# laomao0/BIN

Measured on NVIDIA H100. Metric: 720p frame-windows/sec, higher is better.
Workload: dtype f16

## Files before the change

### bin_b200/build.py

```python
from __future__ import annotations

import hashlib
import os
import subprocess
import sys
import tempfile

HERE = os.path.dirname(os.path.abspath(__file__))
CSRC = os.path.join(HERE, "csrc")
LIB = os.path.join(HERE, "libbin_b200.so")
SOURCES = ["conv_igemm.cu", "rdb_tail.cu", "aux_kernels.cu", "wgrad.cu", "metrics.cu", "png.cu", "api.cu"]
HEADERS = ["common.cuh", "wgmma.cuh", "xstack.cuh", "internal.h", os.path.join("..", "..", "include", "bin_b200.h")]
ARCH = ["-gencode", "arch=compute_90a,code=sm_90a"]
NVCC_FLAGS = [*ARCH, "-lineinfo", "-O3", "-std=c++17", "-Xcompiler", "-fPIC", "--expt-relaxed-constexpr", "-Xptxas", "-v"]


def _nvcc() -> str:
    for cand in (os.environ.get("NVCC"), "/usr/local/cuda/bin/nvcc", "nvcc"):
        if cand and (os.path.isabs(cand) and os.path.exists(cand) or not os.path.isabs(cand)):
            return cand
    raise RuntimeError("nvcc not found")


def _digest() -> str:
    h = hashlib.sha256()
    for f in SOURCES + HEADERS:
        with open(os.path.join(CSRC, f), "rb") as fh:
            h.update(fh.read())
    h.update(" ".join(NVCC_FLAGS).encode())
    return h.hexdigest()


def up_to_date(lib: str = LIB) -> bool:
    stamp = lib + ".sha256"
    return os.path.exists(lib) and os.path.exists(stamp) and open(stamp).read().strip() == _digest()


def build(force: bool = False, verbose: bool = False) -> str:
    stamp = LIB + ".sha256"
    dig = _digest()
    if not force and up_to_date():
        return LIB
    objs = []
    os.makedirs(os.path.join(HERE, "build"), exist_ok=True)
    procs = []
    for src in SOURCES:
        obj = os.path.join(HERE, "build", src.replace(".cu", ".o"))
        cmd = [_nvcc(), *NVCC_FLAGS, "-c", os.path.join(CSRC, src), "-o", obj]
        procs.append((src, subprocess.Popen(cmd, stdout=subprocess.PIPE, stderr=subprocess.STDOUT, text=True)))
        objs.append(obj)
    log = []
    for src, p in procs:
        out, _ = p.communicate()
        log.append(f"== {src}\n{out}")
        if p.returncode != 0:
            sys.stderr.write("\n".join(log))
            raise RuntimeError(f"nvcc failed on {src}")
    fd, tmp = tempfile.mkstemp(prefix=".libbin_b200.", suffix=".so", dir=HERE)
    os.close(fd)
    cmd = [_nvcc(), "-shared", "-o", tmp, *objs, *ARCH]
    r = subprocess.run(cmd, stdout=subprocess.PIPE, stderr=subprocess.STDOUT, text=True)
    log.append(r.stdout)
    if r.returncode != 0:
        os.unlink(tmp)
        sys.stderr.write("\n".join(log))
        raise RuntimeError("link failed")
    os.chmod(tmp, 0o755)
    os.replace(tmp, LIB)
    with open(os.path.join(HERE, "build", "nvcc.log"), "w") as fh:
        fh.write("\n".join(log))
    with open(stamp, "w") as fh:
        fh.write(dig)
    if verbose:
        print("\n".join(log))
    return LIB


if __name__ == "__main__":
    print(build(force="--force" in sys.argv, verbose=True))
```

### bin_b200/csrc/common.cuh

```cuda
#pragma once
#include <cuda.h>
#include <cuda_fp16.h>
#include <cuda_runtime.h>
#include <stdint.h>
#include <stdio.h>

#ifndef BIN_SPIN_LIMIT
#define BIN_SPIN_LIMIT (1u << 27)
#endif

namespace binb {

__device__ __forceinline__ uint32_t smem_u32(const void* p) {
  return static_cast<uint32_t>(__cvta_generic_to_shared(p));
}

__device__ __forceinline__ void mbar_init(uint64_t* bar, uint32_t count) {
  asm volatile("mbarrier.init.shared::cta.b64 [%0], %1;" ::"r"(smem_u32(bar)), "r"(count));
}
__device__ __forceinline__ void fence_barrier_init() {
  asm volatile("fence.mbarrier_init.release.cluster;" ::: "memory");
}
__device__ __forceinline__ void fence_proxy_async() {
  asm volatile("fence.proxy.async.shared::cta;" ::: "memory");
// ... 19 lines not shown
      : "memory");
  return ok != 0;
}
__device__ __forceinline__ void mbar_wait(uint64_t* bar, uint32_t parity) {
  uint32_t spins = 0;
  while (!mbar_try_wait(bar, parity)) {
    if (++spins > BIN_SPIN_LIMIT) {
__trap();
    }
  }
}

__device__ __forceinline__ void tma_prefetch_desc(const void* tmap) {
  asm volatile("prefetch.tensormap [%0];" ::"l"(tmap) : "memory");
}
__device__ __forceinline__ void tma_load_5d(void* smem_dst, const void* tmap, uint64_t* bar, int c0, int c1, int c2,
                                            int c3, int c4) {
  asm volatile(
      "cp.async.bulk.tensor.5d.shared::cluster.global.tile.mbarrier::complete_tx::bytes"
      " [%0], [%1, {%3, %4, %5, %6, %7}], [%2];" ::"r"(smem_u32(smem_dst)),
      "l"(tmap), "r"(smem_u32(bar)), "r"(c0), "r"(c1), "r"(c2), "r"(c3), "r"(c4)
      : "memory");
}
__device__ __forceinline__ void tma_load_4d(void* smem_dst, const void* tmap, uint64_t* bar, int c0, int c1, int c2,
                                            int c3) {
  asm volatile(
      "cp.async.bulk.tensor.4d.shared::cluster.global.tile.mbarrier::complete_tx::bytes"
      " [%0], [%1, {%3, %4, %5, %6}], [%2];" ::"r"(smem_u32(smem_dst)),
      "l"(tmap), "r"(smem_u32(bar)), "r"(c0), "r"(c1), "r"(c2), "r"(c3)
      : "memory");
}
__device__ __forceinline__ void bulk_load_1d(void* smem_dst, const void* gsrc, uint32_t bytes, uint64_t* bar) {
  asm volatile("cp.async.bulk.shared::cluster.global.mbarrier::complete_tx::bytes [%0], [%1], %2, [%3];" ::"r"(
                   smem_u32(smem_dst)),
               "l"(gsrc), "r"(bytes), "r"(smem_u32(bar))
               : "memory");
}

__device__ __forceinline__ uint64_t gmma_desc(uint32_t smem_addr, uint32_t lbo_bytes, uint32_t sbo_bytes) {
  return (uint64_t)((smem_addr >> 4) & 0x3FFFu) | ((uint64_t)((lbo_bytes >> 4) & 0x3FFFu) << 16) |
         ((uint64_t)((sbo_bytes >> 4) & 0x3FFFu) << 32);
}
__device__ __forceinline__ void wgmma_fence() { asm volatile("wgmma.fence.sync.aligned;" ::: "memory"); }
__device__ __forceinline__ void wgmma_commit() { asm volatile("wgmma.commit_group.sync.aligned;" ::: "memory"); }
template <int N>
__device__ __forceinline__ void wgmma_wait() { asm volatile("wgmma.wait_group.sync.aligned %0;" ::"n"(N) : "memory"); }
template <int K>
__device__ __forceinline__ void acc_fence(float (&d)[K]) {
#pragma unroll
  for (int i = 0; i < K; ++i) asm volatile("" : "+f"(d[i])::"memory");
}
__device__ __forceinline__ void wg_sync(int id) { asm volatile("bar.sync %0, 128;" ::"r"(id) : "memory"); }

}
```

### bin_b200/csrc/conv_igemm.cu

```cuda
#include <stdio.h>
#include <stdlib.h>

#include "common.cuh"
#include "internal.h"
#include "wgmma.cuh"
#include "xstack.cuh"

namespace binb {

template <int NT, int KS, bool SX>
struct ConvCfg {
  static constexpr int PAD = KS / 2;
  static constexpr int TW = kTWH - 2 * PAD;
  static constexpr bool ROWSPLIT = (KS == 5);
  static constexpr int ROWS = ROWSPLIT ? kTH : kTH + 2 * PAD;
  static constexpr int A_PLANE = ROWS * kTWH * 16;
  static constexpr int A_BYTES = kKPL * A_PLANE;
  static constexpr int NMMA = SX ? NT * KS : NT;
  static constexpr int TAPS_C = SX ? KS : KS * KS;
  static constexpr int TAPS_S = (SX || ROWSPLIT) ? KS : KS * KS;
  static constexpr int NSUB = ROWSPLIT ? KS : 1;
  static constexpr int W_TAP = kKPL * NMMA * 16;
  static constexpr int W_STAGE = TAPS_S * W_TAP;
  static constexpr int W_CHUNK = TAPS_C * W_TAP;
  static constexpr int XS_BYTES = SX ? kMT * 2 * 2 * kXsFloats<NT> * 4 : 0;
  static_assert(!(SX && ROWSPLIT), "SX is only used for 3x3");
  static_assert(NMMA % 16 == 0 && NMMA <= 256, "invalid wgmma N");
};

struct Ctrl {
  uint64_t full[kMaxStages];
  uint64_t empty[kMaxStages];
  uint64_t wfull[kMaxResidentChunks];
};
static_assert(sizeof(Ctrl) <= 1024, "ctrl block");

__device__ __forceinline__ uint32_t pack_h2(float a, float b) {
  __half2 h = __floats2half2_rn(a, b);
  return *reinterpret_cast<uint32_t*>(&h);
}
__device__ __forceinline__ float2 unpack_h2(uint32_t u) {
  __half2 h = *reinterpret_cast<__half2*>(&u);
  return __half22float2(h);
}

constexpr int kThreads = 384;

constexpr int kPsRowBytes = 4 * 16 + 16;
constexpr int kPsPartBytes = 4 * 8 * kPsRowBytes;
template <bool X3>
constexpr int kPsWarpBytes = (X3 ? 2 : 1) * kPsPartBytes;

__device__ __forceinline__ int x3_plane(int logical_plane) { return 2 * (logical_plane & ~3) + (logical_plane & 3); }
template <bool X3>
__device__ __forceinline__ void store_pair(__half* p, size_t lo_off, float a, float b) {
  if constexpr (X3) {
    const __half h0 = __float2half_rn(a), h1 = __float2half_rn(b);
    const __half2 hh = __halves2half2(h0, h1);
    *reinterpret_cast<__half2*>(p) = hh;
    *reinterpret_cast<__half2*>(p + lo_off) = __floats2half2_rn(a - __half2float(h0), b - __half2float(h1));
  } else {
    *reinterpret_cast<uint32_t*>(p) = pack_h2(a, b);
  }
}

template <int NT, int KS, int EPI, bool SX, bool X3>
__global__ void __launch_bounds__(kThreads, 1) conv_igemm_kernel(const __grid_constant__ ConvParams p) {
  using C = ConvCfg<NT, KS, SX>;
  static_assert(EPI != BIN_EPI_PIXSHUF || NT == 128, "the PixelShuffle staging buffer holds 4 output planes");
  constexpr int NA = C::NMMA / 2;
  auto tile_at = [&](int tq) { return p.reverse ? p.ntiles - 1 - tq : tq; };
  extern __shared__ __align__(1024) uint8_t smem[];
  Ctrl* ctrl = reinterpret_cast<Ctrl*>(smem);
  float* sbias = reinterpret_cast<float*>(smem + 1024);

  const int warp = __shfl_sync(0xffffffffu, threadIdx.x >> 5, 0);
  const int lane = threadIdx.x & 31;
  const uint32_t S = p.nstages;
  const int nchunks = p.nch0 + p.nch1;
  const int nunits = nchunks * C::NSUB;
  const int cps = p.cps;
  const int spt = (nunits + cps - 1) / cps;
  const int unit_bytes = C::A_BYTES + (p.resident ? 0 : C::W_STAGE);
  const int stage_bytes = cps * unit_bytes;
  uint8_t* res_w = smem + kCtrlBytes;
  uint8_t* stage0 = res_w + (p.resident ? nchunks * C::W_CHUNK : 0);

  if (threadIdx.x == 0) {
    tma_prefetch_desc(&p.tmap0);
    if (p.nch1 > 0) tma_prefetch_desc(&p.tmap1);
    for (int i = 0; i < kMaxStages; ++i) {
      mbar_init(&ctrl->full[i], 1);
      mbar_init(&ctrl->empty[i], 8);
    }
    for (int i = 0; i < kMaxResidentChunks; ++i) mbar_init(&ctrl->wfull[i], 1);
    fence_barrier_init();
  }
  const bool bias_in_smem = NT * p.nh <= 256;
  if (bias_in_smem)
    for (int i = threadIdx.x; i < NT * p.nh; i += blockDim.x) sbias[i] = p.bias[i];
  const float* bsrc = bias_in_smem ? sbias : p.bias;
  __syncthreads();

  if (warp == 0) {
    if (lane != 0) return;
    if (p.resident) {
      for (int c = 0; c < nchunks; ++c) {
        mbar_expect_tx(&ctrl->wfull[c], C::W_CHUNK);
        bulk_load_1d(res_w + c * C::W_CHUNK, reinterpret_cast<const uint8_t*>(p.w) + (size_t)c * C::W_CHUNK, C::W_CHUNK,
                     &ctrl->wfull[c]);
      }
    }
    uint32_t s = 0, ph = 0;
    for (int tq = blockIdx.x; tq < p.ntiles; tq += gridDim.x) {
      int t = tile_at(tq);
      const int nh = t % p.nh; t /= p.nh;
      const int txi = t % p.tiles_x; t /= p.tiles_x;
      const int tyi = t % p.tiles_y;
      const int b = p.b0 + t / p.tiles_y;
      const int x0 = txi * C::TW - C::PAD, y0 = p.y0 + tyi * kTH - C::PAD;
      int unit = 0;
      for (int j = 0; j < spt; ++j) {
        const int nu = (nunits - unit < cps) ? nunits - unit : cps;
        mbar_wait(&ctrl->empty[s], ph ^ 1);
        uint8_t* dst = stage0 + (size_t)s * stage_bytes;
        mbar_expect_tx(&ctrl->full[s], (uint32_t)(nu * unit_bytes));
        for (int u = 0; u < nu; ++u) {
          const int c = (unit + u) / C::NSUB, sub = (unit + u) % C::NSUB;
          const int lc = X3 ? c / 3 : c;
          const bool seg1 = lc >= p.nch0l;
          const void* tmap = seg1 ? (const void*)&p.tmap1 : (const void*)&p.tmap0;
          const int lplane = seg1 ? p.plane0_1 + (lc - p.nch0l) * kKPL : p.plane0_0 + lc * kKPL;
          const int plane = X3 ? 2 * lplane + ((c % 3) == 1 ? 4 : 0) : lplane;
          tma_load_4d(dst + (size_t)u * unit_bytes, tmap, &ctrl->full[s], x0 * 8, y0 + (C::ROWSPLIT ? sub : 0), plane, b);
          if (!p.resident) {
            const size_t woff = ((size_t)(nh * nchunks + c) * C::TAPS_C + (C::ROWSPLIT ? sub * KS : 0)) * C::W_TAP;
            bulk_load_1d(dst + (size_t)u * unit_bytes + C::A_BYTES, reinterpret_cast<const uint8_t*>(p.w) + woff,
                         C::W_STAGE, &ctrl->full[s]);
          }
        }
        unit += nu;
        if (++s == S) { s = 0; ph ^= 1; }
      }
    }
    return;
  }
  if (warp < 4) return;

  const int m = (warp - 4) >> 2;
  const int wq = warp & 3;
  const int k4 = lane & 3;
  float* xs = reinterpret_cast<float*>(stage0 + (size_t)S * stage_bytes) + (2 * m + (wq >> 1)) * 2 * kXsFloats<NT>;
  uint8_t* psbuf = stage0 + (size_t)S * stage_bytes + (warp - 4) * kPsWarpBytes<X3>;
  float acc[2][NA];
  constexpr float kAcc = X3 ? (1.f / 256.f) : 1.f;
  uint32_t s = 0, ph = 0;
  auto tile_coords = [&](int tq, int& nh, int& txi, int& tyi, int& b) {
    int t = tile_at(tq);
    nh = t % p.nh; t /= p.nh;
    txi = t % p.tiles_x; t /= p.tiles_x;
    tyi = t % p.tiles_y;
    b = p.b0 + t / p.tiles_y;
  };
  auto pixel = [&](int txi, int tyi, int mb, int h, int& y, int& x) {
    const int L = m * 128 + mb * 64 + wq * 16 + (lane >> 2) + 8 * h;
    const int ty = L >> 5, tx = L & 31;
    y = p.y0 + tyi * kTH + ty; x = txi * C::TW + tx;
    return (tx < C::TW) && (y < p.y0 + p.ny) && (x < p.W);
  };
  for (int tq = blockIdx.x; tq < p.ntiles; tq += gridDim.x) {
    constexpr int NFR = EPI == BIN_EPI_FINAL ? BIN_MAX_FRAMES : 1;
    float fpre[2][2][2][NFR];
    if constexpr (EPI == BIN_EPI_FINAL) {
      int nh, txi, tyi, b;
      tile_coords(tq, nh, txi, tyi, b);
      const int call = b / p.fr.Bc, bb = b % p.fr.Bc;
      const size_t hw = (size_t)p.H * p.W;
#pragma unroll
      for (int mb = 0; mb < 2; ++mb)
#pragma unroll
        for (int h = 0; h < 2; ++h) {
          int y, x;
          const bool valid = pixel(txi, tyi, mb, h, y, x);
#pragma unroll
          for (int e = 0; e < 2; ++e) {
            const int c = 2 * k4 + e;
            const size_t off = ((size_t)bb * 3 + c) * hw + (size_t)y * p.W + x;
#pragma unroll
            for (int fi = 0; fi < NFR; ++fi)
              fpre[mb][h][e][fi] = (valid && c < 3 && fi < p.fr.nframes) ? __ldg(p.fr.frame[call][fi] + off) : 0.f;
          }
        }
    }
    int unit = 0, prev = -1;
    for (int j = 0; j < spt; ++j) {
      const int nu = (nunits - unit < cps) ? nunits - unit : cps;
      mbar_wait(&ctrl->full[s], ph);
      if (p.resident && tq == (int)blockIdx.x) {
        for (int u = 0; u < nu; ++u)
          if ((unit + u) % C::NSUB == 0) mbar_wait(&ctrl->wfull[(unit + u) / C::NSUB], 0);
      }
      const uint32_t st_base = smem_u32(stage0 + (size_t)s * stage_bytes);
      wgmma_fence();
      for (int u = 0; u < nu; ++u) {
        const int c = (unit + u) / C::NSUB, sub = (unit + u) % C::NSUB;
        const uint32_t a_base = st_base + u * unit_bytes;
        const uint32_t w_base = p.resident ? smem_u32(res_w + c * C::W_CHUNK) + (C::ROWSPLIT ? sub * KS * C::W_TAP : 0)
                                           : a_base + C::A_BYTES;
        const uint32_t not_first = (unit + u) != 0 ? 1u : 0u;
#pragma unroll
        for (int tp = 0; tp < C::TAPS_S; ++tp) {
          const int ky = SX ? tp : (C::ROWSPLIT ? 0 : tp / KS);
          const int kx = SX ? 0 : (C::ROWSPLIT ? tp : tp % KS);
#pragma unroll
          for (int jj = 0; jj < kKC / 16; ++jj) {
            const uint64_t bd = gmma_desc(w_base + tp * C::W_TAP + jj * 2 * C::NMMA * 16, C::NMMA * 16, 128);
#pragma unroll
            for (int mb = 0; mb < 2; ++mb) {
              const uint32_t a_row = (uint32_t)(m * 128 + mb * 64 + ky * kTWH + kx);
              const uint64_t ad = gmma_desc(a_base + a_row * 16 + jj * 2 * C::A_PLANE, C::A_PLANE, 128);
              Wgmma<C::NMMA>::mma(acc[mb], ad, bd, (tp == 0 && jj == 0) ? not_first : 1u);
            }
          }
        }
      }
      wgmma_commit();
      wgmma_wait<1>();
      if (prev >= 0 && lane == 0) mbar_arrive(&ctrl->empty[prev]);
      prev = (int)s;
      unit += nu;
      if (++s == S) { s = 0; ph ^= 1; }
    }
    wgmma_wait<0>();
    acc_fence(acc[0]);
    acc_fence(acc[1]);
    if (lane == 0) mbar_arrive(&ctrl->empty[prev]);

    int nh, txi, tyi, b;
    tile_coords(tq, nh, txi, tyi, b);
#pragma unroll
    for (int mb = 0; mb < 2; ++mb) {
      if constexpr (SX) xstack_sum<NT>(acc[mb], xs + mb * kXsFloats<NT>, 3 + 2 * m + (wq >> 1));
#pragma unroll
      for (int h = 0; h < 2; ++h) {
        int y, x;
        const bool valid = pixel(txi, tyi, mb, h, y, x);
        auto val = [&](int i, int e) { return acc[mb][4 * i + 2 * h + e] * kAcc; };
        if constexpr (EPI == BIN_EPI_P8) {
          if (valid) {
            constexpr int NR = SX ? 1 : NT / 8;
            uint32_t rres[NR][X3 ? 2 : 1];
            if (!SX && p.res != nullptr) {
#pragma unroll
              for (int i = 0; i < NR; ++i) {
                const int rel = (nh * NT) / 8 + i;
                if (rel >= p.store_planes) continue;
                const int lp = p.res_plane0 + rel;
                const size_t off = ((((size_t)b * p.res_planes + (X3 ? x3_plane(lp) : lp)) * p.H + y) * p.W + x) * 8 + 2 * k4;
                rres[i][0] = *reinterpret_cast<const uint32_t*>(p.res + off);
                if constexpr (X3) rres[i][X3 ? 1 : 0] = *reinterpret_cast<const uint32_t*>(p.res + off + (size_t)4 * p.H * p.W * 8);
              }
            }
#pragma unroll
            for (int i = 0; i < NT / 8; ++i) {
              const int rel = (nh * NT) / 8 + i;
              if (rel >= p.store_planes) continue;
              const int n = nh * NT + 8 * i + 2 * k4;
              float f0 = val(i, 0) + bsrc[n], f1 = val(i, 1) + bsrc[n + 1];
              if (p.relu) { f0 = fmaxf(f0, 0.f); f1 = fmaxf(f1, 0.f); }
              if (!SX && p.res != nullptr) {
                const float2 g = unpack_h2(rres[SX ? 0 : i][0]);
                f0 += g.x; f1 += g.y;
                if constexpr (X3) {
                  const float2 g2 = unpack_h2(rres[SX ? 0 : i][X3 ? 1 : 0]);
                  f0 += g2.x; f1 += g2.y;
                }
              }
              const int op = p.out_plane0 + rel;
              const size_t off = ((((size_t)b * p.out_planes + (X3 ? x3_plane(op) : op)) * p.H + y) * p.W + x) * 8 + 2 * k4;
              store_pair<X3>(p.out + off, (size_t)4 * p.H * p.W * 8, f0, f1);
            }
          }
        } else if constexpr (EPI == BIN_EPI_PIXSHUF) {
          const int r = lane >> 2;
#pragma unroll
          for (int i = 0; i < NT / 8; ++i) {
#pragma unroll
            for (int e = 0; e < 2; ++e) {
              const int n = nh * NT + 8 * i + 2 * k4 + e;
              const float a = val(i, e) + sbias[n];
              const __half hi = __float2half_rn(a);
              __half* dst = reinterpret_cast<__half*>(psbuf + ((i >> 2) * 8 + r) * kPsRowBytes + (2 * (k4 & 1) + e) * 16) +
                            2 * (i & 3) + (k4 >> 1);
              dst[0] = hi;
              if constexpr (X3) dst[kPsPartBytes / 2] = __float2half_rn(a - __half2float(hi));
            }
          }
          __syncwarp();
          if (valid) {
            const int H2 = 2 * p.H, W2 = 2 * p.W;
            const int yy = 2 * y + (k4 >> 1), xx = 2 * x + (k4 & 1);
#pragma unroll
            for (int q = 0; q < NT / 32; ++q) {
              const int op = p.out_plane0 + nh * (NT / 32) + q;
              const size_t off = ((((size_t)b * p.out_planes + (X3 ? x3_plane(op) : op)) * H2 + yy) * W2 + xx) * 8;
#pragma unroll
              for (int part = 0; part < (X3 ? 2 : 1); ++part)
                *reinterpret_cast<uint4*>(p.out + off + (size_t)part * 4 * H2 * W2 * 8) =
                    *reinterpret_cast<const uint4*>(psbuf + part * kPsPartBytes + (q * 8 + r) * kPsRowBytes + k4 * 16);
            }
          }
          __syncwarp();
        } else {
          if (valid && k4 < 2) {
            const int call = b / p.fr.Bc, bb = b % p.fr.Bc;
            const size_t hw = (size_t)p.H * p.W;
#pragma unroll
            for (int e = 0; e < 2; ++e) {
              const int c = 2 * k4 + e;
              if (c >= 3) continue;
              const size_t off = ((size_t)bb * 3 + c) * hw + (size_t)y * p.W + x;
              float fm = fpre[mb][h][e][0];
#pragma unroll
              for (int fi = 1; fi < NFR; ++fi)
                if (fi < p.fr.nframes) fm += fpre[mb][h][e][fi];
              p.fr.out[call][off] = (val(0, e) + sbias[c]) + fm / (float)p.fr.nframes;
            }
          }
        }
      }
    }
  }
}

typedef CUresult (*EncodeTiledFn)(CUtensorMap*, CUtensorMapDataType, cuuint32_t, void*, const cuuint64_t*,
                                  const cuuint64_t*, const cuuint32_t*, const cuuint32_t*, CUtensorMapInterleave,
                                  CUtensorMapSwizzle, CUtensorMapL2promotion, CUtensorMapFloatOOBfill);

static EncodeTiledFn get_encode_fn() {
  static EncodeTiledFn fn = []() -> EncodeTiledFn {
    void* ptr = nullptr;
    cudaDriverEntryPointQueryResult q;
    if (cudaGetDriverEntryPoint("cuTensorMapEncodeTiled", &ptr, cudaEnableDefault, &q) != cudaSuccess ||
        q != cudaDriverEntryPointSuccess)
      return nullptr;
    return reinterpret_cast<EncodeTiledFn>(ptr);
  }();
  return fn;
}

int make_p8_tmap(CUtensorMap* m, const bin_act_t& t, int box_rows) {
  EncodeTiledFn fn = get_encode_fn();
  if (!fn) return fail(BIN_ERR_CUDA, "cuTensorMapEncodeTiled not available from the driver");
  if ((reinterpret_cast<uintptr_t>(t.ptr) & 15) != 0) return fail(BIN_ERR_ARG, "P8 tensor not 16-byte aligned");
  cuuint64_t dims[4] = {(cuuint64_t)t.W * 8, (cuuint64_t)t.H, (cuuint64_t)t.planes, (cuuint64_t)t.B};
  cuuint64_t strides[3] = {(cuuint64_t)t.W * 16, (cuuint64_t)t.H * t.W * 16, (cuuint64_t)t.planes * t.H * t.W * 16};
  cuuint32_t box[4] = {(cuuint32_t)kTWH * 8, (cuuint32_t)box_rows, (cuuint32_t)kKPL, 1};
  cuuint32_t estr[4] = {1, 1, 1, 1};
  CUresult r = fn(m, CU_TENSOR_MAP_DATA_TYPE_FLOAT16, 4, t.ptr, dims, strides, box, estr,
                  CU_TENSOR_MAP_INTERLEAVE_NONE, CU_TENSOR_MAP_SWIZZLE_NONE, CU_TENSOR_MAP_L2_PROMOTION_L2_256B,
                  CU_TENSOR_MAP_FLOAT_OOB_FILL_NONE);
  if (r != CUDA_SUCCESS) return fail(BIN_ERR_CUDA, "cuTensorMapEncodeTiled failed with code " + std::to_string((int)r));
  return BIN_OK;
}

int make_p8_tmap_box(CUtensorMap* m, const bin_act_t& t, int box_px, int box_rows, int box_planes) {
  EncodeTiledFn fn = get_encode_fn();
  if (!fn) return fail(BIN_ERR_CUDA, "cuTensorMapEncodeTiled not available from the driver");
  if ((reinterpret_cast<uintptr_t>(t.ptr) & 15) != 0) return fail(BIN_ERR_ARG, "P8 tensor not 16-byte aligned");
  if (box_px * 8 > 256 || box_rows > 256 || box_planes > 256) return fail(BIN_ERR_ARG, "TMA box dimension exceeds 256");
  cuuint64_t dims[4] = {(cuuint64_t)t.W * 8, (cuuint64_t)t.H, (cuuint64_t)t.planes, (cuuint64_t)t.B};
  cuuint64_t strides[3] = {(cuuint64_t)t.W * 16, (cuuint64_t)t.H * t.W * 16, (cuuint64_t)t.planes * t.H * t.W * 16};
  cuuint32_t box[4] = {(cuuint32_t)box_px * 8, (cuuint32_t)box_rows, (cuuint32_t)box_planes, 1};
  cuuint32_t estr[4] = {1, 1, 1, 1};
  CUresult r = fn(m, CU_TENSOR_MAP_DATA_TYPE_FLOAT16, 4, t.ptr, dims, strides, box, estr, CU_TENSOR_MAP_INTERLEAVE_NONE,
                  CU_TENSOR_MAP_SWIZZLE_NONE, CU_TENSOR_MAP_L2_PROMOTION_L2_256B, CU_TENSOR_MAP_FLOAT_OOB_FILL_NONE);
  if (r != CUDA_SUCCESS) return fail(BIN_ERR_CUDA, "cuTensorMapEncodeTiled failed with code " + std::to_string((int)r));
  return BIN_OK;
}

template <int NT, int KS, int EPI, bool SX, bool X3>
static int launch_inst(const bin_conv_args_t& a, cudaStream_t s, bool reverse) {
  using C = ConvCfg<NT, KS, SX>;
  ConvParams p;
// ... 78 lines not shown
  const int ny = a.y_count > 0 ? a.y_count : H - a.y_begin;
  if (a.b_begin < 0 || a.y_begin < 0 || a.b_count < 0 || a.y_count < 0 || nb < 1 || ny < 1 || a.b_begin + nb > B ||
      a.y_begin + ny > H)
    return fail(BIN_ERR_ARG, "conv: batch/row sub-range outside the tensor");
  if (a.epilogue != BIN_EPI_P8 && (a.relu || a.res.ptr))
    return fail(BIN_ERR_ARG, "conv: the pixel-shuffle and final epilogues take no ReLU and no residual");
  const bool sx = a.ksize == 3 && a.cout_pad == 32 && a.variant == BIN_CONV_DEFAULT;
  if (a.epilogue == BIN_EPI_P8) {
    const int nstore = a.store_planes > 0 ? a.store_planes : a.cout_pad / 8;
    if (a.out.H != H || a.out.W != W || a.out.B != B || nstore > a.cout_pad / 8 || plane_end(a.out_plane0, nstore) > a.out.planes)
      return fail(BIN_ERR_ARG, "conv: output tensor geometry mismatch");
    if (a.res.ptr && (a.res.H != H || a.res.W != W || a.res.B != B || plane_end(a.res_plane0, nstore) > a.res.planes))
      return fail(BIN_ERR_ARG, "conv: residual tensor geometry mismatch");
    if (sx && a.res.ptr) return fail(BIN_ERR_ARG, "conv: the x-stacked 3x3 / Cout 32 kernel takes no residual");
  } else if (a.epilogue == BIN_EPI_PIXSHUF) {
    if (a.out.H != 2 * H || a.out.W != 2 * W || a.out.B != B || plane_end(a.out_plane0, a.cout_pad / 32) > a.out.planes)
      return fail(BIN_ERR_ARG, "conv: pixel-shuffle output geometry mismatch");
    if (misaligned(a.out.ptr)) return fail(BIN_ERR_ARG, "conv: P8 tensor not 16-byte aligned");
  } else if (a.epilogue == BIN_EPI_FINAL) {
    if (a.fr.ncalls < 1 || a.fr.ncalls > BIN_MAX_CALLS || a.fr.nframes < 1 || a.fr.nframes > BIN_MAX_FRAMES ||
        a.fr.Bc < 1 || a.fr.ncalls * a.fr.Bc != B)
      return fail(BIN_ERR_ARG, "conv: frame table does not match the batch");
  }
  if (!a.in0.ptr || (has_in1 && !a.in1.ptr)) return fail(BIN_ERR_ARG, "conv: null input tensor");
  if (misaligned(a.in0.ptr) || (has_in1 && misaligned(a.in1.ptr))) return fail(BIN_ERR_ARG, "conv: P8 tensor not 16-byte aligned");
  if (!a.w_packed || !a.bias) return fail(BIN_ERR_ARG, "conv: null weights or bias");
  if (a.epilogue != BIN_EPI_FINAL && !a.out.ptr) return fail(BIN_ERR_ARG, "conv: null output tensor");
  if (a.epilogue == BIN_EPI_FINAL)
    for (int k = 0; k < a.fr.ncalls; ++k) {
      bool ok = a.fr.out[k] != nullptr;
      for (int fi = 0; fi < a.fr.nframes; ++fi) ok = ok && a.fr.frame[k][fi] != nullptr;
      if (!ok) return fail(BIN_ERR_ARG, "conv: null frame or output pointer in the frame table");
    }
  if (a.epilogue == BIN_EPI_P8) {
    if (sx) return launch_inst<32, 3, BIN_EPI_P8, true, X3>(a, s, reverse);
    if (a.ksize == 3 && a.cout_pad == 32 && a.variant == BIN_CONV_PLAIN && !X3) return launch_inst<32, 3, BIN_EPI_P8, false, false>(a, s, reverse);
    if (a.ksize == 3 && a.cout_pad % 96 == 0) return launch_inst<96, 3, BIN_EPI_P8, false, X3>(a, s, reverse);
    if (a.ksize == 5 && a.cout_pad == 96) return launch_inst<96, 5, BIN_EPI_P8, false, X3>(a, s, reverse);
    if (a.ksize == 1 && a.cout_pad % 96 == 0) return launch_inst<96, 1, BIN_EPI_P8, false, X3>(a, s, reverse);
  } else if (a.epilogue == BIN_EPI_PIXSHUF) {
    if (a.ksize == 3 && a.cout_pad == 256) return launch_inst<128, 3, BIN_EPI_PIXSHUF, false, X3>(a, s, reverse);
  } else if (a.epilogue == BIN_EPI_FINAL) {
    if (a.ksize == 3 && a.cout_pad == 16 && a.variant == BIN_CONV_DEFAULT) return launch_inst<16, 3, BIN_EPI_FINAL, true, X3>(a, s, reverse);
    if (a.ksize == 3 && a.cout_pad == 16 && a.variant == BIN_CONV_PLAIN && !X3) return launch_inst<16, 3, BIN_EPI_FINAL, false, false>(a, s, reverse);
  }
  return fail(BIN_ERR_UNSUPPORTED, "conv: no kernel instantiation for this conv (ksize/cout_pad/epilogue/precision)");
}

int launch_conv(const bin_conv_args_t& a, cudaStream_t s, bool reverse) {
  return a.x3 ? launch_conv_t<true>(a, s, reverse) : launch_conv_t<false>(a, s, reverse);
}

}
```

### bin_b200/csrc/rdb_tail.cu

```cuda
#include <stdio.h>
#include <stdlib.h>

#include "common.cuh"
#include "internal.h"
#include "wgmma.cuh"
#include "xstack.cuh"

namespace binb {

constexpr int kRtTH = 4;
constexpr int kRtRows = kRtTH + 2;
constexpr int kRtTW = kTWH - 2;
constexpr int kRtAPlane = kRtRows * kTWH * 16;
constexpr int kRtABytes = kKPL * kRtAPlane;
constexpr int kRtN = 96;
constexpr int kRtSlab = kKPL * kRtN * 16;
constexpr int kRtChunks = 6;
constexpr int kRtWChunk = 4 * kRtSlab;
constexpr int kRtWBytes = kRtChunks * kRtWChunk + kRtSlab;
constexpr int kRtHPlane = 128 * 16;
constexpr int kRtHBytes = kKPL * kRtHPlane;
constexpr int kRtXsBytes = 4 * kXsFloats<32> * 4;
constexpr int kRtCtrl = 1024;
constexpr int kRtStages = (kSmemMax - kRtCtrl - kRtWBytes - kRtHBytes - kRtXsBytes) / kRtABytes;
constexpr int kRtSmem = kRtCtrl + kRtWBytes + kRtHBytes + kRtStages * kRtABytes + kRtXsBytes;
static_assert(kRtStages >= 2 && kRtSmem <= kSmemMax, "rdb_tail shared memory");
static_assert((kRtCtrl + kRtWBytes + kRtHBytes) % 128 == 0 && kRtABytes % 128 == 0, "TMA destinations must be 128-byte aligned");

struct alignas(64) RdbTailParams {
  CUtensorMap tmap0, tmap1;
  int plane0_0, plane0_1;
  const uint8_t* w_conv;
  const uint8_t* w_lff;
  const float* b_conv;
  const float* b_lff;
  int H, W;
  int b0, y0, ny;
  int tiles_x, tiles_y, ntiles;
  __half* out; int out_planes, out_plane0;
  const __half* res; int res_planes, res_plane0;
  int reverse;
};

struct RtCtrl {
  uint64_t full[kRtStages], empty[kRtStages];
  uint64_t wfull[kRtChunks + 1];
};
static_assert(sizeof(RtCtrl) <= 512, "ctrl block");

__device__ __forceinline__ uint32_t pack_h2_rt(float a, float b) {
  __half2 h = __floats2half2_rn(a, b);
  return *reinterpret_cast<uint32_t*>(&h);
}
__device__ __forceinline__ float2 unpack_h2_rt(uint32_t u) {
  __half2 h = *reinterpret_cast<__half2*>(&u);
  return __half22float2(h);
}

__global__ void __launch_bounds__(384, 1) rdb_tail_kernel(const __grid_constant__ RdbTailParams p) {
  extern __shared__ __align__(1024) uint8_t smem[];
  RtCtrl* ctrl = reinterpret_cast<RtCtrl*>(smem);
  float* sb_conv = reinterpret_cast<float*>(smem + 512);
  float* sb_lff = sb_conv + 32;
  uint8_t* res_w = smem + kRtCtrl;
  uint8_t* htile = res_w + kRtWBytes;
  uint8_t* stage0 = htile + kRtHBytes;
  float* xs0 = reinterpret_cast<float*>(stage0 + kRtStages * kRtABytes);

  const int warp = __shfl_sync(0xffffffffu, threadIdx.x >> 5, 0);
  const int lane = threadIdx.x & 31;
  auto tile_of = [&](int tq, int& txi, int& tyi, int& b) {
    int t = p.reverse ? p.ntiles - 1 - tq : tq;
    txi = t % p.tiles_x; t /= p.tiles_x;
    tyi = t % p.tiles_y;
    b = p.b0 + t / p.tiles_y;
  };

  if (threadIdx.x == 0) {
    tma_prefetch_desc(&p.tmap0);
    tma_prefetch_desc(&p.tmap1);
    for (int i = 0; i < kRtStages; ++i) { mbar_init(&ctrl->full[i], 1); mbar_init(&ctrl->empty[i], 8); }
    for (int i = 0; i <= kRtChunks; ++i) mbar_init(&ctrl->wfull[i], 1);
    fence_barrier_init();
  }
  if (threadIdx.x < 32) sb_conv[threadIdx.x] = p.b_conv[threadIdx.x];
  else if (threadIdx.x < 128) sb_lff[threadIdx.x - 32] = p.b_lff[threadIdx.x - 32];
  __syncthreads();

  if (warp == 0) {
    if (lane != 0) return;
    for (int c = 0; c < kRtChunks; ++c) {
      mbar_expect_tx(&ctrl->wfull[c], kRtWChunk);
      bulk_load_1d(res_w + c * kRtWChunk, p.w_conv + (size_t)c * 3 * kRtSlab, 3 * kRtSlab, &ctrl->wfull[c]);
      bulk_load_1d(res_w + c * kRtWChunk + 3 * kRtSlab, p.w_lff + (size_t)c * kRtSlab, kRtSlab, &ctrl->wfull[c]);
    }
    mbar_expect_tx(&ctrl->wfull[kRtChunks], kRtSlab);
    bulk_load_1d(res_w + kRtChunks * kRtWChunk, p.w_lff + (size_t)kRtChunks * kRtSlab, kRtSlab, &ctrl->wfull[kRtChunks]);
    uint32_t s = 0, ph = 0;
    for (int tq = blockIdx.x; tq < p.ntiles; tq += gridDim.x) {
      int txi, tyi, b;
      tile_of(tq, txi, tyi, b);
      const int x0 = txi * kRtTW - 1, y0 = p.y0 + tyi * kRtTH - 1;
      for (int c = 0; c < kRtChunks; ++c) {
        mbar_wait(&ctrl->empty[s], ph ^ 1);
        mbar_expect_tx(&ctrl->full[s], kRtABytes);
        const bool seg1 = c >= 3;
        tma_load_4d(stage0 + (size_t)s * kRtABytes, seg1 ? (const void*)&p.tmap1 : (const void*)&p.tmap0, &ctrl->full[s],
                    x0 * 8, y0, seg1 ? p.plane0_1 + (c - 3) * kKPL : p.plane0_0 + c * kKPL, b);
        if (++s == kRtStages) { s = 0; ph ^= 1; }
      }
    }
    return;
  }
  if (warp < 4) return;

  const int m = (warp - 4) >> 2;
  const int wq = warp & 3;
  const int k4 = lane & 3;
  float* xs = xs0 + (2 * m + (wq >> 1)) * kXsFloats<32>;
  const int xs_bar = 3 + 2 * m + (wq >> 1);
  float acc_c[kRtN / 2], acc_l[kRtN / 2];
  uint32_t s = 0, ph = 0;
  for (int tq = blockIdx.x; tq < p.ntiles; tq += gridDim.x) {
    int prev = -1;
    for (int c = 0; c < kRtChunks; ++c) {
      mbar_wait(&ctrl->full[s], ph);
      if (tq == (int)blockIdx.x) mbar_wait(&ctrl->wfull[c], 0);
      const uint32_t a_base = smem_u32(stage0 + (size_t)s * kRtABytes) + m * 64 * 16;
      const uint32_t b_base = smem_u32(res_w + c * kRtWChunk);
      const uint32_t first = c == 0 ? 0u : 1u;
      wgmma_fence();
#pragma unroll
      for (int ky = 0; ky < 3; ++ky) {
#pragma unroll
        for (int jj = 0; jj < kKC / 16; ++jj)
          Wgmma<kRtN>::mma(acc_c, gmma_desc(a_base + ky * kTWH * 16 + jj * 2 * kRtAPlane, kRtAPlane, 128),
                           gmma_desc(b_base + ky * kRtSlab + jj * 2 * kRtN * 16, kRtN * 16, 128),
                           (jj == 0 && ky == 0) ? first : 1u);
      }
#pragma unroll
      for (int jj = 0; jj < kKC / 16; ++jj)
        Wgmma<kRtN>::mma(acc_l, gmma_desc(a_base + (kTWH + 1) * 16 + jj * 2 * kRtAPlane, kRtAPlane, 128),
                         gmma_desc(b_base + 3 * kRtSlab + jj * 2 * kRtN * 16, kRtN * 16, 128), jj == 0 ? first : 1u);
      wgmma_commit();
      wgmma_wait<1>();
      if (prev >= 0 && lane == 0) mbar_arrive(&ctrl->empty[prev]);
      prev = (int)s;
      if (++s == kRtStages) { s = 0; ph ^= 1; }
    }
    wgmma_wait<0>();
    acc_fence(acc_c);
    acc_fence(acc_l);
    if (lane == 0) mbar_arrive(&ctrl->empty[prev]);

    int txi, tyi, b;
    tile_of(tq, txi, tyi, b);
    bool valid[2];
    int y[2], x[2];
    uint32_t res[2][kRtN / 8];
#pragma unroll
    for (int h = 0; h < 2; ++h) {
      const int L = m * 64 + wq * 16 + (lane >> 2) + 8 * h;
      y[h] = p.y0 + tyi * kRtTH + (L >> 5);
      x[h] = txi * kRtTW + (L & 31);
      valid[h] = (L & 31) < kRtTW && y[h] < p.y0 + p.ny && x[h] < p.W;
#pragma unroll
      for (int i = 0; i < kRtN / 8; ++i) {
        const size_t roff = ((((size_t)b * p.res_planes + p.res_plane0 + i) * p.H + y[h]) * p.W + x[h]) * 8 + 2 * k4;
        res[h][i] = valid[h] ? *reinterpret_cast<const uint32_t*>(p.res + roff) : 0u;
      }
    }

    xstack_sum<32>(acc_c, xs, xs_bar);
#pragma unroll
    for (int h = 0; h < 2; ++h) {
      const int r = wq * 16 + (lane >> 2) + 8 * h;
      uint8_t* hrow = htile + (m * 64 + r) * 16 + 4 * k4;
#pragma unroll
      for (int i = 0; i < 4; ++i) {
        float f[2];
#pragma unroll
        for (int e = 0; e < 2; ++e) f[e] = fmaxf(acc_c[4 * i + 2 * h + e] + sb_conv[8 * i + 2 * k4 + e], 0.f);
        *reinterpret_cast<uint32_t*>(hrow + i * kRtHPlane) = pack_h2_rt(f[0], f[1]);
      }
    }
    fence_proxy_async();
    wg_sync(1 + m);

    if (tq == (int)blockIdx.x) mbar_wait(&ctrl->wfull[kRtChunks], 0);
    wgmma_fence();
    {
      const uint32_t h_base = smem_u32(htile) + m * 64 * 16;
      const uint32_t b_base = smem_u32(res_w + kRtChunks * kRtWChunk);
#pragma unroll
      for (int jj = 0; jj < kKC / 16; ++jj)
        Wgmma<kRtN>::mma(acc_l, gmma_desc(h_base + jj * 2 * kRtHPlane, kRtHPlane, 128),
                         gmma_desc(b_base + jj * 2 * kRtN * 16, kRtN * 16, 128), 1u);
    }
    wgmma_commit();
    wgmma_wait<0>();
    acc_fence(acc_l);

#pragma unroll
    for (int h = 0; h < 2; ++h) {
      if (valid[h]) {
#pragma unroll
        for (int i = 0; i < kRtN / 8; ++i) {
          const int n = 8 * i + 2 * k4;
          const float2 g = unpack_h2_rt(res[h][i]);
          const size_t off = ((((size_t)b * p.out_planes + p.out_plane0 + i) * p.H + y[h]) * p.W + x[h]) * 8 + 2 * k4;
          *reinterpret_cast<uint32_t*>(p.out + off) =
              pack_h2_rt((acc_l[4 * i + 2 * h] + sb_lff[n]) + g.x, (acc_l[4 * i + 2 * h + 1] + sb_lff[n + 1]) + g.y);
        }
      }
    }
    wg_sync(1 + m);
  }
}

int make_p8_tmap(CUtensorMap* m, const bin_act_t& t, int box_rows);

int launch_rdb_tail(const bin_act_t& x, int x_plane0, const bin_act_t& g, int g_plane0, const void* w_conv,
                    const float* b_conv, const void* w_lff, const float* b_lff, const bin_act_t& out, int out_plane0,
                    int b_begin, int b_count, int y_begin, int y_count, cudaStream_t s, bool reverse) {
  const int H = x.H, W = x.W, B = x.B;
  if (g.H != H || g.W != W || g.B != B || out.H != H || out.W != W || out.B != B)
    return fail(BIN_ERR_ARG, "rdb_tail: tensor geometry mismatch");
  if (x_plane0 < 0 || g_plane0 < 0 || out_plane0 < 0 || x_plane0 + 12 > x.planes || g_plane0 + 12 > g.planes ||
      out_plane0 + 12 > out.planes)
    return fail(BIN_ERR_ARG, "rdb_tail: plane range exceeds tensor");
  RdbTailParams p;
  memset(&p, 0, sizeof(p));
  p.plane0_0 = x_plane0; p.plane0_1 = g_plane0;
  p.w_conv = reinterpret_cast<const uint8_t*>(w_conv); p.w_lff = reinterpret_cast<const uint8_t*>(w_lff);
  p.b_conv = b_conv; p.b_lff = b_lff;
  p.H = H; p.W = W;
  p.b0 = b_begin; p.y0 = y_begin;
  const int nb = b_count > 0 ? b_count : B - b_begin;
  p.ny = y_count > 0 ? y_count : H - y_begin;
  if (p.b0 < 0 || p.y0 < 0 || nb < 1 || p.ny < 1 || p.b0 + nb > B || p.y0 + p.ny > H)
    return fail(BIN_ERR_ARG, "rdb_tail: batch/row sub-range outside the tensor");
  if (!x.ptr || !g.ptr || !out.ptr || !w_conv || !b_conv || !w_lff || !b_lff) return fail(BIN_ERR_ARG, "rdb_tail_fwd: null argument");
  p.tiles_x = (W + kRtTW - 1) / kRtTW;
  p.tiles_y = (p.ny + kRtTH - 1) / kRtTH;
  p.ntiles = nb * p.tiles_x * p.tiles_y;
  p.out = reinterpret_cast<__half*>(out.ptr); p.out_planes = out.planes; p.out_plane0 = out_plane0;
  p.res = reinterpret_cast<const __half*>(x.ptr); p.res_planes = x.planes; p.res_plane0 = x_plane0;
  p.reverse = reverse ? 1 : 0;
  BIN_TRY(make_p8_tmap(&p.tmap0, x, kRtRows));
  BIN_TRY(make_p8_tmap(&p.tmap1, g, kRtRows));
  static std::atomic<unsigned long long> opted{0};
  BIN_TRY(ensure_dynamic_smem(rdb_tail_kernel, kRtSmem, opted));
  const int sms = num_sms();
  const int grid = p.ntiles < sms ? p.ntiles : sms;
  rdb_tail_kernel<<<grid, 384, kRtSmem, s>>>(p);
  BIN_CUDA_OK(cudaGetLastError());
  return BIN_OK;
}

}
```

Before: 15.51.

## Overlap next-tile conv head with RDB tail epilogue and read residual from smem

In the RDB tail kernel, the first two conv chunks of the next tile are issued before waiting on the LFF GEMM, so tensor-core work overlaps the epilogue stores. The residual is read from the staged TMA input tile in shared memory instead of a separate global load. Both kernels also hand registers from producer to consumer warpgroups with setmaxnreg. Optional clock64 phase instrumentation is added behind a compile flag, along with a build helper for instrumented libraries. This adds ring-slot ordering constraints and raises register pressure in the consumers.

New measurement: 16.70, median of 6. 1.08x the previous value.

```diff
diff --git a/bin_b200/build.py b/bin_b200/build.py
--- a/bin_b200/build.py
+++ b/bin_b200/build.py
@@ -36,17 +36,13 @@
     return os.path.exists(lib) and os.path.exists(stamp) and open(stamp).read().strip() == _digest()
 
 
-def build(force: bool = False, verbose: bool = False) -> str:
-    stamp = LIB + ".sha256"
-    dig = _digest()
-    if not force and up_to_date():
-        return LIB
+def _compile_link(lib: str, obj_dir: str, extra_flags: list) -> str:
     objs = []
-    os.makedirs(os.path.join(HERE, "build"), exist_ok=True)
+    os.makedirs(obj_dir, exist_ok=True)
     procs = []
     for src in SOURCES:
-        obj = os.path.join(HERE, "build", src.replace(".cu", ".o"))
-        cmd = [_nvcc(), *NVCC_FLAGS, "-c", os.path.join(CSRC, src), "-o", obj]
+        obj = os.path.join(obj_dir, src.replace(".cu", ".o"))
+        cmd = [_nvcc(), *NVCC_FLAGS, *extra_flags, "-c", os.path.join(CSRC, src), "-o", obj]
         procs.append((src, subprocess.Popen(cmd, stdout=subprocess.PIPE, stderr=subprocess.STDOUT, text=True)))
         objs.append(obj)
     log = []
@@ -56,7 +52,7 @@
         if p.returncode != 0:
             sys.stderr.write("\n".join(log))
             raise RuntimeError(f"nvcc failed on {src}")
-    fd, tmp = tempfile.mkstemp(prefix=".libbin_b200.", suffix=".so", dir=HERE)
+    fd, tmp = tempfile.mkstemp(prefix=".libbin_b200.", suffix=".so", dir=os.path.dirname(lib))
     os.close(fd)
     cmd = [_nvcc(), "-shared", "-o", tmp, *objs, *ARCH]
     r = subprocess.run(cmd, stdout=subprocess.PIPE, stderr=subprocess.STDOUT, text=True)
@@ -66,14 +62,29 @@
         sys.stderr.write("\n".join(log))
         raise RuntimeError("link failed")
     os.chmod(tmp, 0o755)
-    os.replace(tmp, LIB)
+    os.replace(tmp, lib)
+    return "\n".join(log)
+
+
+def build(force: bool = False, verbose: bool = False) -> str:
+    stamp = LIB + ".sha256"
+    dig = _digest()
+    if not force and up_to_date():
+        return LIB
+    log = _compile_link(LIB, os.path.join(HERE, "build"), [])
     with open(os.path.join(HERE, "build", "nvcc.log"), "w") as fh:
-        fh.write("\n".join(log))
+        fh.write(log)
     with open(stamp, "w") as fh:
         fh.write(dig)
     if verbose:
-        print("\n".join(log))
+        print(log)
     return LIB
+
+
+def build_instrumented(out_dir: str, defines: list) -> str:
+    lib = os.path.join(out_dir, "libbin_b200_" + "_".join(d.lower() for d in defines) + ".so")
+    _compile_link(lib, os.path.join(out_dir, "obj"), [f"-D{d}" for d in defines])
+    return lib
 
 
 if __name__ == "__main__":
diff --git a/bin_b200/csrc/common.cuh b/bin_b200/csrc/common.cuh
--- a/bin_b200/csrc/common.cuh
+++ b/bin_b200/csrc/common.cuh
@@ -95,4 +95,22 @@
 }
 __device__ __forceinline__ void wg_sync(int id) { asm volatile("bar.sync %0, 128;" ::"r"(id) : "memory"); }
 
+constexpr int kProducerRegs = 40;
+constexpr int kConsumerRegs = 232;
+template <int R>
+__device__ __forceinline__ void setmaxnreg_dec() { asm volatile("setmaxnreg.dec.sync.aligned.u32 %0;" ::"n"(R)); }
+template <int R>
+__device__ __forceinline__ void setmaxnreg_inc() { asm volatile("setmaxnreg.inc.sync.aligned.u32 %0;" ::"n"(R)); }
+
+#ifdef BIN_RDB_PHASES
+#define BIN_PH(...) __VA_ARGS__
+struct PhaseBuf {
+  unsigned long long* rec;
+  int max_tiles;
+};
+enum { PH_START, PH_LAST_FULL, PH_MMA_DONE, PH_EPI_DONE, PH_STARVED_MAIN, PH_STARVED_EPI, kPhTile = 8 };
+#else
+#define BIN_PH(...)
+#endif
+
 }
diff --git a/bin_b200/csrc/conv_igemm.cu b/bin_b200/csrc/conv_igemm.cu
--- a/bin_b200/csrc/conv_igemm.cu
+++ b/bin_b200/csrc/conv_igemm.cu
@@ -44,6 +44,10 @@
   return __half22float2(h);
 }
 
+#ifdef BIN_RDB_PHASES
+static __device__ PhaseBuf g_ph_conv;
+#endif
+
 constexpr int kThreads = 384;
 
 constexpr int kPsRowBytes = 4 * 16 + 16;
@@ -68,6 +72,7 @@
 __global__ void __launch_bounds__(kThreads, 1) conv_igemm_kernel(const __grid_constant__ ConvParams p) {
   using C = ConvCfg<NT, KS, SX>;
   static_assert(EPI != BIN_EPI_PIXSHUF || NT == 128, "the PixelShuffle staging buffer holds 4 output planes");
+  constexpr bool kRdb = SX && EPI == BIN_EPI_P8;
   constexpr int NA = C::NMMA / 2;
   auto tile_at = [&](int tq) { return p.reverse ? p.ntiles - 1 - tq : tq; };
   extern __shared__ __align__(1024) uint8_t smem[];
@@ -102,8 +107,10 @@
   const float* bsrc = bias_in_smem ? sbias : p.bias;
   __syncthreads();
 
-  if (warp == 0) {
-    if (lane != 0) return;
+  if (warp < 4) {
+    if constexpr (kRdb) setmaxnreg_dec<kProducerRegs>();
+    if (warp != 0 || lane != 0) return;
+    BIN_PH(unsigned long long blocked = 0, ntq = 0;)
     if (p.resident) {
       for (int c = 0; c < nchunks; ++c) {
         mbar_expect_tx(&ctrl->wfull[c], C::W_CHUNK);
@@ -122,7 +129,9 @@
       int unit = 0;
       for (int j = 0; j < spt; ++j) {
         const int nu = (nunits - unit < cps) ? nunits - unit : cps;
+        BIN_PH(const unsigned long long w0 = clock64();)
         mbar_wait(&ctrl->empty[s], ph ^ 1);
+        BIN_PH(blocked += clock64() - w0;)
         uint8_t* dst = stage0 + (size_t)s * stage_bytes;
         mbar_expect_tx(&ctrl->full[s], (uint32_t)(nu * unit_bytes));
         for (int u = 0; u < nu; ++u) {
@@ -142,10 +151,15 @@
         unit += nu;
         if (++s == S) { s = 0; ph ^= 1; }
       }
-    }
+      BIN_PH(++ntq;)
+    }
+    BIN_PH(if (kRdb && g_ph_conv.rec) {
+      g_ph_conv.rec[2 * (size_t)g_ph_conv.max_tiles * kPhTile + 2 * blockIdx.x] = blocked;
+      g_ph_conv.rec[2 * (size_t)g_ph_conv.max_tiles * kPhTile + 2 * blockIdx.x + 1] = ntq;
+    })
     return;
   }
-  if (warp < 4) return;
+  if constexpr (kRdb) setmaxnreg_inc<kConsumerRegs>();
 
   const int m = (warp - 4) >> 2;
   const int wq = warp & 3;
@@ -168,7 +182,10 @@
     y = p.y0 + tyi * kTH + ty; x = txi * C::TW + tx;
     return (tx < C::TW) && (y < p.y0 + p.ny) && (x < p.W);
   };
+  BIN_PH(const bool rec = kRdb && wq == 0 && lane == 0 && g_ph_conv.rec != nullptr;
+         unsigned long long starved = 0, starved_main = 0, t_start = 0, t_last_full = 0, t_mma = 0;)
   for (int tq = blockIdx.x; tq < p.ntiles; tq += gridDim.x) {
+    BIN_PH(t_start = clock64();)
     constexpr int NFR = EPI == BIN_EPI_FINAL ? BIN_MAX_FRAMES : 1;
     float fpre[2][2][2][NFR];
     if constexpr (EPI == BIN_EPI_FINAL) {
@@ -195,11 +212,13 @@
     int unit = 0, prev = -1;
     for (int j = 0; j < spt; ++j) {
       const int nu = (nunits - unit < cps) ? nunits - unit : cps;
+      BIN_PH(const unsigned long long w0 = clock64();)
       mbar_wait(&ctrl->full[s], ph);
       if (p.resident && tq == (int)blockIdx.x) {
         for (int u = 0; u < nu; ++u)
           if ((unit + u) % C::NSUB == 0) mbar_wait(&ctrl->wfull[(unit + u) / C::NSUB], 0);
       }
+      BIN_PH(starved += clock64() - w0;)
       const uint32_t st_base = smem_u32(stage0 + (size_t)s * stage_bytes);
       wgmma_fence();
       for (int u = 0; u < nu; ++u) {
@@ -231,10 +250,12 @@
       unit += nu;
       if (++s == S) { s = 0; ph ^= 1; }
     }
+    BIN_PH(t_last_full = clock64();)
     wgmma_wait<0>();
     acc_fence(acc[0]);
     acc_fence(acc[1]);
     if (lane == 0) mbar_arrive(&ctrl->empty[prev]);
+    BIN_PH(t_mma = clock64(); starved_main = starved; starved = 0;)
 
     int nh, txi, tyi, b;
     tile_coords(tq, nh, txi, tyi, b);
@@ -330,6 +351,11 @@
         }
       }
     }
+    BIN_PH(if (rec && tq < g_ph_conv.max_tiles) {
+      unsigned long long* r = g_ph_conv.rec + (2 * (size_t)tq + m) * kPhTile;
+      r[PH_START] = t_start; r[PH_LAST_FULL] = t_last_full; r[PH_MMA_DONE] = t_mma; r[PH_EPI_DONE] = clock64();
+      r[PH_STARVED_MAIN] = starved_main; r[PH_STARVED_EPI] = starved;
+    } starved = 0;)
   }
 }
 
@@ -514,3 +540,10 @@
 }
 
 }
+
+#ifdef BIN_RDB_PHASES
+extern "C" int bin_rdb_phases_arm_conv(void* rec, int max_tiles) {
+  const binb::PhaseBuf b{reinterpret_cast<unsigned long long*>(rec), max_tiles};
+  return cudaMemcpyToSymbol(binb::g_ph_conv, &b, sizeof(b)) == cudaSuccess ? BIN_OK : BIN_ERR_CUDA;
+}
+#endif
diff --git a/bin_b200/csrc/rdb_tail.cu b/bin_b200/csrc/rdb_tail.cu
--- a/bin_b200/csrc/rdb_tail.cu
+++ b/bin_b200/csrc/rdb_tail.cu
@@ -16,6 +16,7 @@
 constexpr int kRtN = 96;
 constexpr int kRtSlab = kKPL * kRtN * 16;
 constexpr int kRtChunks = 6;
+constexpr int kRtXChunks = 3;
 constexpr int kRtWChunk = 4 * kRtSlab;
 constexpr int kRtWBytes = kRtChunks * kRtWChunk + kRtSlab;
 constexpr int kRtHPlane = 128 * 16;
@@ -25,6 +26,9 @@
 constexpr int kRtStages = (kSmemMax - kRtCtrl - kRtWBytes - kRtHBytes - kRtXsBytes) / kRtABytes;
 constexpr int kRtSmem = kRtCtrl + kRtWBytes + kRtHBytes + kRtStages * kRtABytes + kRtXsBytes;
 static_assert(kRtStages >= 2 && kRtSmem <= kSmemMax, "rdb_tail shared memory");
+constexpr int kRtHead = 2;
+static_assert(kRtHead >= 1 && kRtHead < kRtChunks && kRtHead <= kRtStages,
+              "the head's ring slots must be released by the main loop of the tile before");
 static_assert((kRtCtrl + kRtWBytes + kRtHBytes) % 128 == 0 && kRtABytes % 128 == 0, "TMA destinations must be 128-byte aligned");
 
 struct alignas(64) RdbTailParams {
@@ -38,7 +42,6 @@
   int b0, y0, ny;
   int tiles_x, tiles_y, ntiles;
   __half* out; int out_planes, out_plane0;
-  const __half* res; int res_planes, res_plane0;
   int reverse;
 };
 
@@ -56,6 +59,10 @@
   __half2 h = *reinterpret_cast<__half2*>(&u);
   return __half22float2(h);
 }
+
+#ifdef BIN_RDB_PHASES
+static __device__ PhaseBuf g_ph_tail;
+#endif
 
 __global__ void __launch_bounds__(384, 1) rdb_tail_kernel(const __grid_constant__ RdbTailParams p) {
   extern __shared__ __align__(1024) uint8_t smem[];
@@ -87,8 +94,10 @@
   else if (threadIdx.x < 128) sb_lff[threadIdx.x - 32] = p.b_lff[threadIdx.x - 32];
   __syncthreads();
 
-  if (warp == 0) {
-    if (lane != 0) return;
+  if (warp < 4) {
+    setmaxnreg_dec<kProducerRegs>();
+    if (warp != 0 || lane != 0) return;
+    BIN_PH(unsigned long long blocked = 0, ntq = 0;)
     for (int c = 0; c < kRtChunks; ++c) {
       mbar_expect_tx(&ctrl->wfull[c], kRtWChunk);
       bulk_load_1d(res_w + c * kRtWChunk, p.w_conv + (size_t)c * 3 * kRtSlab, 3 * kRtSlab, &ctrl->wfull[c]);
@@ -102,17 +111,24 @@
       tile_of(tq, txi, tyi, b);
       const int x0 = txi * kRtTW - 1, y0 = p.y0 + tyi * kRtTH - 1;
       for (int c = 0; c < kRtChunks; ++c) {
+        BIN_PH(const unsigned long long w0 = clock64();)
         mbar_wait(&ctrl->empty[s], ph ^ 1);
+        BIN_PH(blocked += clock64() - w0;)
         mbar_expect_tx(&ctrl->full[s], kRtABytes);
-        const bool seg1 = c >= 3;
+        const bool seg1 = c >= kRtXChunks;
         tma_load_4d(stage0 + (size_t)s * kRtABytes, seg1 ? (const void*)&p.tmap1 : (const void*)&p.tmap0, &ctrl->full[s],
-                    x0 * 8, y0, seg1 ? p.plane0_1 + (c - 3) * kKPL : p.plane0_0 + c * kKPL, b);
+                    x0 * 8, y0, seg1 ? p.plane0_1 + (c - kRtXChunks) * kKPL : p.plane0_0 + c * kKPL, b);
         if (++s == kRtStages) { s = 0; ph ^= 1; }
       }
-    }
+      BIN_PH(++ntq;)
+    }
+    BIN_PH(if (g_ph_tail.rec) {
+      g_ph_tail.rec[2 * (size_t)g_ph_tail.max_tiles * kPhTile + 2 * blockIdx.x] = blocked;
+      g_ph_tail.rec[2 * (size_t)g_ph_tail.max_tiles * kPhTile + 2 * blockIdx.x + 1] = ntq;
+    })
     return;
   }
-  if (warp < 4) return;
+  setmaxnreg_inc<kConsumerRegs>();
 
   const int m = (warp - 4) >> 2;
   const int wq = warp & 3;
@@ -121,54 +137,90 @@
   const int xs_bar = 3 + 2 * m + (wq >> 1);
   float acc_c[kRtN / 2], acc_l[kRtN / 2];
   uint32_t s = 0, ph = 0;
+  BIN_PH(const bool rec = wq == 0 && lane == 0 && g_ph_tail.rec != nullptr;
+         unsigned long long starved = 0, starved_main = 0, t_start = 0, t_last_full = 0, t_mma = 0;)
+  auto a_base_of = [&](uint32_t slot) { return smem_u32(stage0 + (size_t)slot * kRtABytes) + m * 64 * 16; };
+  auto conv_mma = [&](uint32_t a_base, int c) {
+    const uint32_t b_base = smem_u32(res_w + c * kRtWChunk);
+#pragma unroll
+    for (int ky = 0; ky < 3; ++ky)
+#pragma unroll
+      for (int jj = 0; jj < kKC / 16; ++jj)
+        Wgmma<kRtN>::mma(acc_c, gmma_desc(a_base + ky * kTWH * 16 + jj * 2 * kRtAPlane, kRtAPlane, 128),
+                         gmma_desc(b_base + ky * kRtSlab + jj * 2 * kRtN * 16, kRtN * 16, 128),
+                         (jj == 0 && ky == 0 && c == 0) ? 0u : 1u);
+  };
+  auto issue_head = [&](bool exists, bool first_tile) {
+    uint32_t hs = s, hph = ph;
+#pragma unroll
+    for (int c = 0; c < kRtHead; ++c) {
+      if (exists) {
+        BIN_PH(const unsigned long long w0 = clock64();)
+        mbar_wait(&ctrl->full[hs], hph);
+        if (first_tile) mbar_wait(&ctrl->wfull[c], 0);
+        BIN_PH(starved += clock64() - w0;)
+      }
+      wgmma_fence();
+      conv_mma(a_base_of(hs), c);
+      if (++hs == kRtStages) { hs = 0; hph ^= 1; }
+    }
+    wgmma_commit();
+  };
+
+  issue_head(true, true);
   for (int tq = blockIdx.x; tq < p.ntiles; tq += gridDim.x) {
+    const bool first_tile = tq == (int)blockIdx.x;
+    BIN_PH(t_start = clock64();)
+    uint32_t res[2][kRtN / 8];
     int prev = -1;
+#pragma unroll
     for (int c = 0; c < kRtChunks; ++c) {
-      mbar_wait(&ctrl->full[s], ph);
-      if (tq == (int)blockIdx.x) mbar_wait(&ctrl->wfull[c], 0);
-      const uint32_t a_base = smem_u32(stage0 + (size_t)s * kRtABytes) + m * 64 * 16;
+      if (c >= kRtHead) {
+        BIN_PH(const unsigned long long w0 = clock64();)
+        mbar_wait(&ctrl->full[s], ph);
+        if (first_tile) mbar_wait(&ctrl->wfull[c], 0);
+        BIN_PH(starved += clock64() - w0;)
+      }
+      const uint32_t a_base = a_base_of(s);
+      wgmma_fence();
+      if (c >= kRtHead) conv_mma(a_base, c);
       const uint32_t b_base = smem_u32(res_w + c * kRtWChunk);
-      const uint32_t first = c == 0 ? 0u : 1u;
-      wgmma_fence();
-#pragma unroll
-      for (int ky = 0; ky < 3; ++ky) {
-#pragma unroll
-        for (int jj = 0; jj < kKC / 16; ++jj)
-          Wgmma<kRtN>::mma(acc_c, gmma_desc(a_base + ky * kTWH * 16 + jj * 2 * kRtAPlane, kRtAPlane, 128),
-                           gmma_desc(b_base + ky * kRtSlab + jj * 2 * kRtN * 16, kRtN * 16, 128),
-                           (jj == 0 && ky == 0) ? first : 1u);
-      }
 #pragma unroll
       for (int jj = 0; jj < kKC / 16; ++jj)
         Wgmma<kRtN>::mma(acc_l, gmma_desc(a_base + (kTWH + 1) * 16 + jj * 2 * kRtAPlane, kRtAPlane, 128),
-                         gmma_desc(b_base + 3 * kRtSlab + jj * 2 * kRtN * 16, kRtN * 16, 128), jj == 0 ? first : 1u);
+                         gmma_desc(b_base + 3 * kRtSlab + jj * 2 * kRtN * 16, kRtN * 16, 128), (jj == 0 && c == 0) ? 0u : 1u);
       wgmma_commit();
+      if (c < kRtXChunks) {
+#pragma unroll
+        for (int h = 0; h < 2; ++h)
+#pragma unroll
+          for (int j = 0; j < kKPL; ++j)
+            res[h][kKPL * c + j] = *reinterpret_cast<const uint32_t*>(
+                stage0 + (size_t)s * kRtABytes + (m * 64 + wq * 16 + (lane >> 2) + 8 * h + kTWH + 1) * 16 + j * kRtAPlane + 4 * k4);
+      }
       wgmma_wait<1>();
+      if (c >= 1 && c <= kRtXChunks) __syncwarp();
       if (prev >= 0 && lane == 0) mbar_arrive(&ctrl->empty[prev]);
       prev = (int)s;
       if (++s == kRtStages) { s = 0; ph ^= 1; }
     }
+    BIN_PH(t_last_full = clock64();)
     wgmma_wait<0>();
     acc_fence(acc_c);
     acc_fence(acc_l);
     if (lane == 0) mbar_arrive(&ctrl->empty[prev]);
+    BIN_PH(t_mma = clock64(); starved_main = starved; starved = 0;)
 
     int txi, tyi, b;
     tile_of(tq, txi, tyi, b);
     bool valid[2];
     int y[2], x[2];
-    uint32_t res[2][kRtN / 8];
 #pragma unroll
     for (int h = 0; h < 2; ++h) {
       const int L = m * 64 + wq * 16 + (lane >> 2) + 8 * h;
       y[h] = p.y0 + tyi * kRtTH + (L >> 5);
       x[h] = txi * kRtTW + (L & 31);
       valid[h] = (L & 31) < kRtTW && y[h] < p.y0 + p.ny && x[h] < p.W;
-#pragma unroll
-      for (int i = 0; i < kRtN / 8; ++i) {
-        const size_t roff = ((((size_t)b * p.res_planes + p.res_plane0 + i) * p.H + y[h]) * p.W + x[h]) * 8 + 2 * k4;
-        res[h][i] = valid[h] ? *reinterpret_cast<const uint32_t*>(p.res + roff) : 0u;
-      }
     }
 
     xstack_sum<32>(acc_c, xs, xs_bar);
@@ -187,7 +239,11 @@
     fence_proxy_async();
     wg_sync(1 + m);
 
-    if (tq == (int)blockIdx.x) mbar_wait(&ctrl->wfull[kRtChunks], 0);
+    if (first_tile) {
+      BIN_PH(const unsigned long long w0 = clock64();)
+      mbar_wait(&ctrl->wfull[kRtChunks], 0);
+      BIN_PH(starved += clock64() - w0;)
+    }
     wgmma_fence();
     {
       const uint32_t h_base = smem_u32(htile) + m * 64 * 16;
@@ -198,7 +254,8 @@
                          gmma_desc(b_base + jj * 2 * kRtN * 16, kRtN * 16, 128), 1u);
     }
     wgmma_commit();
-    wgmma_wait<0>();
+    issue_head(tq + (int)gridDim.x < p.ntiles, false);
+    wgmma_wait<1>();
     acc_fence(acc_l);
 
 #pragma unroll
@@ -215,7 +272,16 @@
       }
     }
     wg_sync(1 + m);
+    BIN_PH(if (rec) {
+      unsigned long long* r = g_ph_tail.rec + (2 * (size_t)tq + m) * kPhTile;
+      if (tq < g_ph_tail.max_tiles) {
+        r[PH_START] = t_start; r[PH_LAST_FULL] = t_last_full; r[PH_MMA_DONE] = t_mma; r[PH_EPI_DONE] = clock64();
+        r[PH_STARVED_MAIN] = starved_main; r[PH_STARVED_EPI] = starved;
+      }
+      starved = 0;
+    })
   }
+  wgmma_wait<0>();
 }
 
 int make_p8_tmap(CUtensorMap* m, const bin_act_t& t, int box_rows);
@@ -245,7 +311,6 @@
   p.tiles_y = (p.ny + kRtTH - 1) / kRtTH;
   p.ntiles = nb * p.tiles_x * p.tiles_y;
   p.out = reinterpret_cast<__half*>(out.ptr); p.out_planes = out.planes; p.out_plane0 = out_plane0;
-  p.res = reinterpret_cast<const __half*>(x.ptr); p.res_planes = x.planes; p.res_plane0 = x_plane0;
   p.reverse = reverse ? 1 : 0;
   BIN_TRY(make_p8_tmap(&p.tmap0, x, kRtRows));
   BIN_TRY(make_p8_tmap(&p.tmap1, g, kRtRows));
@@ -259,3 +324,10 @@
 }
 
 }
+
+#ifdef BIN_RDB_PHASES
+extern "C" int bin_rdb_phases_arm_tail(void* rec, int max_tiles) {
+  const binb::PhaseBuf b{reinterpret_cast<unsigned long long*>(rec), max_tiles};
+  return cudaMemcpyToSymbol(binb::g_ph_tail, &b, sizeof(b)) == cudaSuccess ? BIN_OK : BIN_ERR_CUDA;
+}
+#endif
```
